# yxtay/transformer-recommenders

Hardware: AMD Instinct MI355X
Metric: user-sequences/sec (train step) MovieLens-1M seq200 d128 @1/2/4/8 GPU (higher is better)
Workload: dtype bf16; 1 GPU; MovieLens-1M-shaped: 3883 items, seq_len=200, d_model=128, 4-layer causal BERT (heads=4, ffn=512), InfoNCELoss over in-batch shared negatives, AdamW; per_gpu_batch=512, global_batch=512, seq_len=200, lengths=dense, loss_heads_evaluated=all 7 + LogitsStatistics (reference training_step), parallelism=dp1, launch=eager launches

## Files before the change

### transformer-recommenders_amd/csrc/common.h

```cpp
#pragma once
#include <hip/hip_runtime.h>
#include <stdint.h>

#include "xfmr_hip.h"

typedef __attribute__((ext_vector_type(8))) __bf16 bf16x8;
typedef __attribute__((ext_vector_type(4))) __bf16 bf16x4;
typedef __attribute__((ext_vector_type(2))) __bf16 bf16x2;
typedef __attribute__((ext_vector_type(16))) float f32x16;

#define XF_WAVE 64

#define XF_LAUNCH_CHECK()                                   \
  do {                                                      \
    if (hipGetLastError() != hipSuccess) return XFMR_EHIP;  \
  } while (0)

static inline bool xf_aligned16(const void* p) { return (reinterpret_cast<uintptr_t>(p) & 15u) == 0; }

__device__ __forceinline__ int xf_lane() { return threadIdx.x & 63; }

__device__ __forceinline__ int xf_acc_row(int r, int lane) { return (r & 3) + 8 * (r >> 2) + 4 * (lane >> 5); }

struct PrecBF16 {
// ... 503 lines not shown
  }
  __device__ static __forceinline__ void tile_xb_tr(f32x16& acc, const __bf16* img, int hsub, int jrow0,
                                                    const f32x16& x) {
    const int l = xf_lane(), g16 = l >> 4, hh = g16 >> 1, li = l & 15, q = li >> 2, p = li & 3;
    const int col = hsub * 32 + 16 * (g16 & 1) + 4 * p;
    const int c = col >> 3, within = col & 7;
#pragma unroll
    for (int s = 0; s < 2; ++s) {
      bf16x8 b;
#pragma unroll
      for (int j = 0; j < 8; ++j) b[j] = (__bf16)x[8 * s + j];
      union { xf_s16x4 v[2]; bf16x8 f; } a;
#pragma unroll
      for (int t = 0; t < 2; ++t) {
        const int row = jrow0 + 16 * s + 8 * t + 4 * hh + q;
        const __bf16* ptr = img + off(row, c) + within;
        a.v[t] = __builtin_amdgcn_ds_read_tr16_b64_v4i16(
            (__attribute__((address_space(3))) xf_s16x4*)(ptr));
      }
      acc = __builtin_amdgcn_mfma_f32_32x32x16_bf16(a.f, b, acc, 0, 0, 0);
    }
  }
  __device__ static __forceinline__ bf16x8 frag_tr(const __bf16* img, int col0, int k0) {
    const int l = xf_lane(), g16 = l >> 4, li = l & 15, q = li >> 2, p = li & 3;
    const int col = col0 + 16 * (g16 & 1) + 4 * p;
    const int c = col >> 3, within = col & 7;
    union { xf_s16x4 v[2]; bf16x8 f; } a;
#pragma unroll
    for (int t = 0; t < 2; ++t) {
      const int row = k0 + 8 * (g16 >> 1) + 4 * t + q;
      a.v[t] = __builtin_amdgcn_ds_read_tr16_b64_v4i16(
          (__attribute__((address_space(3))) xf_s16x4*)(img + off(row, c) + within));
    }
    return a.f;
  }
  __device__ static __forceinline__ int gather_row(int row0) { return row0 + xf_lane() / CPR; }
  __device__ static __forceinline__ int gather_src_chunk(int row) { return (xf_lane() % CPR) ^ swz(row); }
  static constexpr int kRowsPerInstr = 64 / CPR;
};

__device__ __forceinline__ void xf_glds16(const void* gsrc, void* lds_base) {
  __builtin_amdgcn_global_load_lds((const __attribute__((address_space(1))) void*)gsrc,
                                   (__attribute__((address_space(3))) void*)lds_base, 16, 0, 0);
}
__device__ __forceinline__ void xf_glds16_raw_so(const void* sbase, uint32_t voff, void* lds_base) {
  const unsigned dst = (unsigned)(uintptr_t)(__attribute__((address_space(3))) void*)lds_base;
  unsigned keep;
// ... 18 lines not shown
```

### transformer-recommenders_amd/csrc/encoder.hip

```cpp
#include <math.h>
#include <stdlib.h>
#include <new>
#include <string.h>

#include "internal.h"

namespace {

struct LayerParams {
  int64_t wqkv, bqkv, wo, bo, ln1g, ln1b, w1, b1, w2, b2, ln2g, ln2b;
};
struct ParamLayout {
  int64_t pos, type, eg, eb;
  int64_t total;
};

int64_t layer_base(const xfmr_encoder_cfg* c, int i, ParamLayout* pl) {
  const int64_t H = c->hidden, I = c->inter;
  pl->pos = 0;
  pl->type = pl->pos + (int64_t)c->max_pos * H;
  pl->eg = pl->type + 2 * H;
  pl->eb = pl->eg + H;
  const int64_t first = pl->eb + H;
  const int64_t per = 3 * H * H + 3 * H + H * H + H + 2 * H + I * H + I + H * I + H + 2 * H;
// ... 45 lines not shown
size_t up256(size_t x) { return (x + 255) & ~(size_t)255; }

__global__ __launch_bounds__(256) void params_to_bf16_kernel(const float* src, __bf16* dst, int64_t n4) {
  const int64_t i = (int64_t)blockIdx.x * 256 + threadIdx.x;
  if (i < n4) xf_st4<true>(dst, 4 * i, *reinterpret_cast<const float4*>(src + 4 * i));
}

bool mixed_storage(const xfmr_encoder_cfg* c) {
  static const bool force_fp32 = [] {
    const char* e = getenv("XFMR_ACT_FP32");
    return e && *e && *e != '0';
  }();
  return c->precision == XFMR_PREC_BF16 && !force_fp32;
}
int prof(const xfmr_encoder_cfg* c, int kind, int layer, int which, hipStream_t st) {
  if (c->profile_kernel != kind || c->profile_layer != layer || !c->profile_events[which]) return XFMR_OK;
  return hipEventRecord((hipEvent_t)c->profile_events[which], st) == hipSuccess ? XFMR_OK : XFMR_EHIP;
}

struct EncPlan {
  int64_t Tplan, T;
  bool mix, causal;
  bool fuse_ln, fuse_ffn, rederive, fuse_ffn_bwd, dw_buffers_per_layer, dw_side, group_dw, lin_copy;
  int half_layer;
};
constexpr int64_t kDwSideTokens = 40960;
constexpr int64_t kFfnFusedTokens = 16384;
int64_t ln_fused_min_tokens() {
  static const int64_t min_tokens = [] { const char* e = getenv("XFMR_LN_FUSED_MIN_TOKENS"); return e ? (int64_t)atoll(e) : (int64_t)12288; }();
  return min_tokens;
}
EncPlan make_plan(const xfmr_encoder_cfg* c) {
  EncPlan p{};
  const uint32_t f = c->flags;
  p.Tplan = (int64_t)c->batch * c->seq_len;
  p.T = c->seq_offsets ? c->packed_rows : p.Tplan;
  p.mix = mixed_storage(c);
  p.causal = !(f & XFMR_ENC_BIDIRECTIONAL);
  p.fuse_ln = p.mix && c->hidden == 128 && p.Tplan >= ln_fused_min_tokens() && !(f & XFMR_ENC_LN_UNFUSED);
  p.fuse_ffn = p.fuse_ln && p.Tplan >= kFfnFusedTokens && (c->inter % 128) == 0 && c->inter <= 1024 && !(f & XFMR_ENC_FFN_UNFUSED);
  const char* const store_x = getenv("XFMR_LN_STORE_X");
  p.rederive = p.fuse_ln && !(store_x && *store_x && *store_x != '0');
  p.fuse_ffn_bwd = p.fuse_ffn && p.fuse_ln && !(f & XFMR_ENC_FFN_BWD_UNFUSED);
  const bool side_any = (f & XFMR_ENC_DW_SIDE_ANY) != 0;
  p.dw_buffers_per_layer = p.mix && c->layers <= 64 && (side_any || (c->hidden == 128 && p.Tplan >= kDwSideTokens)) &&
                           c->context && !(f & XFMR_ENC_DW_INLINE);
  p.dw_side = p.dw_buffers_per_layer && (side_any || p.T >= kDwSideTokens || !c->seq_offsets);
  p.group_dw = !(f & XFMR_ENC_DW_UNPAIRED) && !p.dw_side && p.mix;
  p.lin_copy = c->hidden_dropout > 0.f || p.mix;
  p.half_layer = ((c->grads_half_event || (f & XFMR_ENC_REDUCE_HALF_EARLY)) && c->layers >= 2) ? c->layers / 2 : -1;
  return p;
}

struct Bump {
  unsigned char* base;
  size_t o;
  void* bytes(size_t n) { void* p = base ? base + o : nullptr; o += up256(n); return p; }
  float* f32(size_t n) { return reinterpret_cast<float*>(bytes(n * sizeof(float))); }
};
struct Workspace {
  Acts a;
  unsigned char* base;
  int layers;
  bool per_layer;
  size_t T, TH, TI, lse, es, xb, slab_w2, slab_w1, slab_wo, slab_wqkv, b1, bqkv, lnrec;
  size_t grads0, grads_stride, red0, red_stride, act0, act_stride;
// ... 221 lines not shown
int xfmr_context_destroy(void* context) {
  if (!context) return XFMR_EINVAL;
  XfContext* c = (XfContext*)context;
  if (c->ev_in) (void)hipEventDestroy(c->ev_in);
  if (c->ev_done) (void)hipEventDestroy(c->ev_done);
  if (c->side) (void)hipStreamDestroy(c->side);
  delete c;
  return XFMR_OK;
}

}

namespace {

struct Residual { const float* x; XfLnResidual re; };

int encoder_forward(const xfmr_encoder_cfg* cfg, const EncPlan& plan, const FwdBufs& a, const float* params,
                    const int64_t* item_idx, const float* table, int64_t n_rows, float* tok, uint8_t* key_mask, hipStream_t st) {
  const int B = cfg->batch, L = cfg->seq_len, H = cfg->hidden, I = cfg->inter, A = cfg->heads;
  const int32_t* const offs = cfg->seq_offsets;
  const int64_t T = plan.T;
  const int prec = cfg->precision;
  const bool mix = plan.mix, keep = a.keep, rederive = plan.rederive && keep;
  const float hdrop = cfg->hidden_dropout, eps = cfg->ln_eps;
  const XfSeed sd(cfg->seed, keep ? cfg->step_device : nullptr);
  ParamLayout pl;
  layer_base(cfg, 0, &pl);
  float* const x0 = rederive ? nullptr : a.x0;
  if (offs) {
    XF_TRY(xf_embed_ln_fwd_packed_ex(item_idx, table, n_rows, params + pl.pos, params + pl.type, params + pl.eg,
                                     params + pl.eb, x0, mix ? a.x0b : nullptr, a.emb_pre, a.emb_mean, a.emb_rstd, key_mask,
                                     T, cfg->row_pos, H, eps, hdrop, sd, SITE_EMB, st));
  } else {
    XF_TRY(xf_embed_ln_fwd_ex(item_idx, table, n_rows, params + pl.pos, params + pl.type, params + pl.eg,
                              params + pl.eb, x0, mix ? a.x0b : nullptr, a.emb_pre, a.emb_mean, a.emb_rstd, key_mask, B,
                              L, H, eps, hdrop, sd, SITE_EMB, st));
  }
  if (cfg->embed_event && hipEventRecord((hipEvent_t)cfg->embed_event, st) != hipSuccess) return XFMR_EHIP;
  Residual x{x0, {a.emb_pre, a.emb_mean, a.emb_rstd, params + pl.eg, params + pl.eb, hdrop, SITE_EMB}};
  const void* xg = mix ? a.x0b : (const void*)a.x0;
  if (mix) {
    const int64_t n4 = pl.total / 4;
    hipLaunchKernelGGL(params_to_bf16_kernel, dim3((unsigned)((n4 + 255) / 256)), dim3(256), 0, st, params,
                       (__bf16*)a.wbf, n4);
    XF_LAUNCH_CHECK();
  }
// ... 15 lines not shown
    float* const sum = keep ? pre : a.ln_tmp;
    XF_TRY(xf_linear_fwd_ex(in, W(w), params + bias, sum, T, H, K, XFMR_EPI_BIAS_DROP_RES, res.x, nullptr, hdrop, sd, site,
                            prec, sA | sB, st));
    return xf_layernorm_fwd_ex(sum, params + gamma, params + beta, y, y16, mean, rstd, T, H, eps, st);
  };
  for (int i = 0; i < cfg->layers; ++i) {
    const LayerActs l = a.layer(i);
    const LayerParams p = layer_params(cfg, i);
    const bool last = i == cfg->layers - 1;
    float* const x1 = rederive ? nullptr : l.x1;
    float* const out = last ? tok : (rederive ? nullptr : l.x2);
    void* const x1b = mix ? l.x1b : nullptr;
    void* const x2b = (mix && !last) ? l.x2b : nullptr;
    XF_TRY(xf_linear_fwd_ex(xg, W(p.wqkv), params + p.bqkv, l.qkv, T, 3 * H, H, XFMR_EPI_BIAS, nullptr, nullptr,
                            0.f, 0, 0, prec, sC | sA | sB, st));
    XF_TRY(prof(cfg, XFMR_PROF_ATTN_FWD, i, 0, st));
    XF_TRY(xf_attn_fwd_ex(l.qkv, key_mask, l.ctx, l.lse, B, L, A, H, cfg->attn_dropout, sd, site_attn(i), prec,
                          mix, plan.causal, st, offs));
    XF_TRY(prof(cfg, XFMR_PROF_ATTN_FWD, i, 1, st));
    XF_TRY(linear_ln(l.ctx, p.wo, p.bo, H, x, site_out(i), p.ln1g, p.ln1b, l.pre1, x1, x1b, l.mean1, l.rstd1));
    XF_TRY(prof(cfg, XFMR_PROF_FFN_FWD, i, 0, st));
    const Residual r1{x1, {l.pre1, l.mean1, l.rstd1, params + p.ln1g, params + p.ln1b, 0.f, 0}};
    if (plan.fuse_ffn) {
      XF_TRY(rederive ? xf_ffn_fwd_fused_re(l.x1b, W(p.w1), params + p.b1, W(p.w2), params + p.b2, l.f1, l.g, l.pre2, T, H,
                                            I, &r1.re, hdrop, sd, site_ffn(i), params + p.ln2g, params + p.ln2b, eps, out,
                                            x2b, l.mean2, l.rstd2, st)
             : !keep  ? xf_ffn_fwd_fused_infer(l.x1b, W(p.w1), params + p.b1, W(p.w2), params + p.b2, T, H, I, r1.x,
                                               params + p.ln2g, params + p.ln2b, eps, out, x2b, st)
                      : xf_ffn_fwd_fused_ex(l.x1b, W(p.w1), params + p.b1, W(p.w2), params + p.b2, l.f1, l.g, l.pre2, T, H,
                                            I, r1.x, hdrop, sd, site_ffn(i), params + p.ln2g, params + p.ln2b, eps, out,
                                            x2b, l.mean2, l.rstd2, st));
    } else {
      const void* const x1g = mix ? (const void*)l.x1b : (const void*)l.x1;
      if (keep)
        XF_TRY(xf_linear_fwd_ex(x1g, W(p.w1), params + p.b1, l.g, T, I, H, XFMR_EPI_BIAS_GELU, nullptr, l.f1, 0.f, 0, 0, prec,
                                sC | sA | sB | XF_AUX_GELU_GRAD, st));
      else
        XF_TRY(xf_linear_gelu_fwd_infer(x1g, W(p.w1), params + p.b1, l.g, T, I, H, prec, sC | sA | sB, st));
      XF_TRY(linear_ln(l.g, p.w2, p.b2, I, r1, site_ffn(i), p.ln2g, p.ln2b, l.pre2, out, x2b, l.mean2, l.rstd2));
    }
    XF_TRY(prof(cfg, XFMR_PROF_FFN_FWD, i, 1, st));
    x = Residual{out, {l.pre2, l.mean2, l.rstd2, params + p.ln2g, params + p.ln2b, 0.f, 0}};
    xg = mix ? (const void*)l.x2b : (const void*)out;
  }
  return XFMR_OK;
}

}

extern "C" {

int xfmr_encoder_fwd(const xfmr_encoder_cfg* cfg, const float* params, const int64_t* item_idx,
// ... 95 lines not shown
                                   mix, nullptr, nullptr, nullptr, T, H, off,
                                   xf_make_dropout(cfg->hidden_dropout, sd, site_ffn(i)), r.ln2, st, &blocks));
      ln_segs(r.ln2, blocks, p.ln2g, p.ln2b, p.b2);
    }
    const void* const dlin_ffn = lin_copy ? gb.dLinF : (const void*)a.dA;
    const void* const dlin_out = lin_copy ? gb.dLinO : (const void*)dX;
    int splits[4] = {0, 0, 0, 0};
    const XfDwItem items[4] = {
        {dlin_ffn, l.g, (int32_t)H, (int32_t)I, r.w2, nullptr, &splits[0]},
        {gb.dI, mix ? (const void*)l.x1b : (const void*)l.x1, (int32_t)I, (int32_t)H, r.w1, r.b1, &splits[1]},
        {dlin_out, l.ctx, (int32_t)H, (int32_t)H, r.wo, nullptr, &splits[2]},
        {gb.dQKV, i > 0 ? (mix ? prev.x2b : (const void*)prev.x2) : (mix ? a.x0b : (const void*)a.x0), (int32_t)(3 * H),
         (int32_t)H, r.wqkv, r.bqkv, &splits[3]}};
    const int64_t dw_w[4] = {p.w2, p.w1, p.wo, p.wqkv}, dw_b[4] = {-1, p.b1, -1, p.bqkv};
    auto dw = [&](int k, bool launch) -> int {
      const XfDwItem& it = items[k];
      if (launch) XF_TRY(xf_linear_bwd_dw_deferred(it.dy, it.x, T, it.N, it.K, prec, sAB, it.slabs, it.bias_part, it.splits, dw_stream()));
      seg(it.slabs, grads + dw_w[k], *it.splits, (int64_t)it.N * it.K, (int64_t)it.N * it.K);
      if (it.bias_part) seg(it.bias_part, grads + dw_b[k], *it.splits, it.N, it.N);
      return XFMR_OK;
    };
    if (!plan.group_dw) XF_TRY(dw(0, true));
    XF_TRY(prof(cfg, XFMR_PROF_FFN_BWD, i, 0, st));
    if (plan.fuse_ffn_bwd) {
      XF_TRY(xf_ffn_bwd_dx_fused_ex(dlin_ffn, W(p.w2), l.f1, W(p.w1), gb.dI, T, H, I, a.dA, l.pre1, l.mean1, l.rstd1,
                                    params + p.ln1g, cfg->hidden_dropout, sd, site_out(i), dX, gb.dLinO, r.ln1,
                                    &blocks, st));
    } else {
      XF_TRY(xf_linear_bwd_dx_ex(dlin_ffn, W(p.w2), gb.dI, T, H, I, nullptr, l.f1, prec,
                                 sA | sC | sP | sB | (plan.fuse_ffn ? 0 : XF_AUX_GELU_GRAD), st));
    }
    if (!plan.group_dw) XF_TRY(dw(1, true));
    if (plan.fuse_ffn_bwd) {
    } else if (fuse_lnb) {
      XF_TRY(xf_linear_bwd_dx_lnbwd_ex(gb.dI, W(p.w1), T, I, H, a.dA, l.pre1, l.mean1, l.rstd1, params + p.ln1g,
                                       cfg->hidden_dropout, sd, site_out(i), dX, gb.dLinO, r.ln1, &blocks, prec,
                                       sA | sB, st));
    } else {
      XF_TRY(xf_linear_bwd_dx_ex(gb.dI, W(p.w1), a.dA, T, I, H, a.dA, nullptr, prec, sA | sB, st));
      XF_TRY(xf_layernorm_bwd_impl(a.dA, l.pre1, l.mean1, l.rstd1, params + p.ln1g, dX, lin_copy ? gb.dLinO : nullptr,
                                   mix, nullptr, nullptr, nullptr, T, H, off,
                                   xf_make_dropout(cfg->hidden_dropout, sd, site_out(i)), r.ln1, st, &blocks));
    }
    XF_TRY(prof(cfg, XFMR_PROF_FFN_BWD, i, 1, st));
    ln_segs(r.ln1, blocks, p.ln1g, p.ln1b, p.bo);
    if (!plan.group_dw) XF_TRY(dw(2, true));
    XF_TRY(xf_linear_bwd_dx_ex(dlin_out, W(p.wo), a.dCtx, T, H, H, nullptr, nullptr, prec, sA | sC | sB, st));
// ... 38 lines not shown
    XF_TRY(xf_layernorm_bwd_impl(dX, a.emb_pre, a.emb_mean, a.emb_rstd, params + pl.eg, a.dA, nullptr, false, nullptr,
                                 nullptr, nullptr, T, H, xf_make_dropout(cfg->hidden_dropout, sd, SITE_EMB), off,
                                 a.emb_ln, st, &blocks));
    ln_segs(a.emb_ln, blocks, pl.eg, pl.eb, -1);
  }
  if (offs) XF_TRY(xf_embed_param_grads_packed(a.dA, grads + pl.pos, grads + pl.type, offs, B, L, H, cfg->max_pos, st));
  else XF_TRY(xfmr_embed_param_grads(a.dA, grads + pl.pos, grads + pl.type, B, L, H, cfg->max_pos, stream));
  return XFMR_OK;
  }();
  if (side_used) {
    if (hipEventRecord(ev_done, side) != hipSuccess || hipStreamWaitEvent(st, ev_done, 0) != hipSuccess) side_rc = XFMR_EHIP;
  }
  if (chain_rc != XFMR_OK) return chain_rc;
  if (side_rc != XFMR_OK) return side_rc;
  XF_TRY(prof(cfg, XFMR_PROF_REDUCE, cfg->profile_layer, 0, st));
  XF_TRY(xf_multi_rowsum(segs, nseg, st));
  XF_TRY(prof(cfg, XFMR_PROF_REDUCE, cfg->profile_layer, 1, st));
  if (cfg->grads_half_event && plan.half_layer < 0 &&
      hipEventRecord((hipEvent_t)cfg->grads_half_event, st) != hipSuccess)
    return XFMR_EHIP;
  return XFMR_OK;
}

int xf_encoder_plan(const xfmr_encoder_cfg* cfg, int32_t out[16]) {
  XF_TRY(check_cfg(cfg));
  if (!out) return XFMR_EINVAL;
  const EncPlan p = make_plan(cfg);
  const int32_t v[16] = {(int32_t)p.Tplan, (int32_t)p.T, p.mix, p.causal, p.fuse_ln, p.fuse_ffn, p.rederive,
                         p.fuse_ffn_bwd, p.dw_buffers_per_layer, p.dw_side, p.group_dw, p.lin_copy, p.half_layer};
  memcpy(out, v, sizeof(v));
  return XFMR_OK;
}

int64_t xfmr_param_half_offset(const xfmr_encoder_cfg* cfg) {
  if (!cfg || cfg->layers <= 0) return XFMR_EINVAL;
  if (cfg->layers < 2) return 0;
  return layer_params(cfg, cfg->layers / 2).wqkv;
}

}
```

### transformer-recommenders_amd/csrc/gemm.hip

```cpp
#include <stdio.h>
#include <stdlib.h>
#include <string.h>

#include <algorithm>
#include <type_traits>

#include "internal.h"

#define XF_PIN_SCALAR(x) asm volatile("" : "+v"(x))
#ifndef XF_LN_DIAG
#define XF_LN_DIAG 0
#endif
#ifndef XF_GEMM_PF
#define XF_GEMM_PF 1
#endif
#ifndef XF_DW_PF
#define XF_DW_PF 1
#endif
#ifdef XF_FFN_STAMP
#define XF_STAMP(i) do { if (stamp_on) st_buf[(i)] = __builtin_readcyclecounter(); } while (0)
#else
#define XF_STAMP(i) do {} while (0)
#endif
#ifndef XF_FFN_ASM_BARRIER
// ... 1157 lines not shown
      XF_LOOP_BARRIER();
      xf_static_for<2>([&](auto ic) {
        constexpr int i = decltype(ic)::value;
        const int p = tid + i * 256, row = p >> 3, ch = p & 7;
        const bf16x8 d8 = di_piece(sF, i);
        if (m0 + row < M) *reinterpret_cast<bf16x8*>(f.DI + (m0 + row) * I + c * CH + ch * 8) = d8;
        *reinterpret_cast<bf16x8*>(sG + row * LDC + ch * 8) = d8;
      });
      commit_w1();
      XF_LOOP_BARRIER();
      if (c + 1 < nchunk) { load_w1(c + 1); load_u(c + 1); }
#pragma unroll
      for (int ks = 0; ks < CH / 16; ++ks) {
        const bf16x8 fa = FN::get(sG, LDC, wr * 32, ks * 16);
#pragma unroll
        for (int j = 0; j < 2; ++j) accx[j] = xf_mma(fa, FT::get(sW, LD2, wc * 64 + j * 32, ks * 16), accx[j]);
      }
    }
    __syncthreads();
    epi_dx_lnbwd_64x128(accx, reinterpret_cast<unsigned char*>(sW), f.e, m0, tix.m, wid, lane);
  }
}

template <class T>
__global__ __launch_bounds__(256) void rowsum_kernel(float* dst, const T* src, int64_t rows, int64_t cols,
                                                     int64_t rows_per) {
  __shared__ float red[4][64];
  const int c = threadIdx.x & 63, rg = threadIdx.x >> 6;
  const int64_t col = (int64_t)blockIdx.x * 64 + c;
  const int64_t r0 = (int64_t)blockIdx.y * rows_per;
  const int64_t r1 = (r0 + rows_per < rows) ? r0 + rows_per : rows;
  float s0 = 0.f, s1 = 0.f, s2 = 0.f, s3 = 0.f;
  if (col < cols) {
    int64_t r = r0 + rg;
    for (; r + 12 < r1; r += 16) {
      s0 += (float)src[r * cols + col];
      s1 += (float)src[(r + 4) * cols + col];
      s2 += (float)src[(r + 8) * cols + col];
      s3 += (float)src[(r + 12) * cols + col];
    }
    for (; r < r1; r += 4) s0 += (float)src[r * cols + col];
  }
  red[rg][c] = (s0 + s1) + (s2 + s3);
  __syncthreads();
  if (rg == 0 && col < cols) dst[(int64_t)blockIdx.y * cols + col] = (red[0][c] + red[1][c]) + (red[2][c] + red[3][c]);
}
// ... 394 lines not shown
  const GemmPlan p = gemm_plan(GemmKey{kGemmFfnBwd, M, H, I, XFMR_PREC_BF16, 0, 1, xf_num_cus()}, gemm_switches());
  if (const int rc = plan_rc(p, xf_aligned16(dy16) && xf_aligned16(w2_16) && xf_aligned16(u16) && xf_aligned16(w1_16) &&
                                    xf_aligned16(di16) && xf_aligned16(dx) && xf_aligned16(ln_x) && xf_aligned16(residual_grad) &&
                                    xf_aligned16(d_lin16) && xf_aligned16(ln_gamma)))
    return rc;
  FfnBwdArgs f{};
  f.DY = (const __bf16*)dy16; f.W2 = (const __bf16*)w2_16; f.U = (const __bf16*)u16; f.W1 = (const __bf16*)w1_16;
  f.DI = (__bf16*)di16; f.I = I;
  GemmArgs& g = f.e;
  g.C = dx; g.ldc = H; g.M = M; g.N = H; g.K = I; g.R = residual_grad;
  g.drop = xf_make_dropout(dropout_p, seed, site);
  g.drop2 = xf_make_dropout(0.f, 0, 0);
  g.ln_gamma = ln_gamma; g.lnb_x = ln_x; g.lnb_mean = ln_mean; g.lnb_rstd = ln_rstd; g.D16 = d_lin16;
  g.lnb_partials = partials;
  set_tiles(g, p);
  *blocks_out = p.records;
  const dim3 grid((unsigned)p.grid), block((unsigned)p.block);
  if (p.ffn_ring) hipLaunchKernelGGL(ffn_bwd_dx_fused_kernel<true>, grid, block, 0, st, f);
  else hipLaunchKernelGGL(ffn_bwd_dx_fused_kernel<false>, grid, block, 0, st, f);
  XF_LAUNCH_CHECK();
  return XFMR_OK;
}

int xf_linear_bwd_dx_ex(const void* dy, const float* w, void* dx, int64_t M, int32_t N, int32_t K,
                        const float* residual_grad, const void* gelu_pre, int32_t precision, uint32_t s16,
                        hipStream_t st) {
  if (!dy || !w || !dx) return XFMR_EINVAL;
  const GemmKey k{gelu_pre ? kGemmDxGelu : kGemmDx, M, N, K, precision, s16, 1, 0};
  const GemmPlan p = gemm_plan(k, gemm_switches_once());
  if (const int rc = plan_rc(p, xf_aligned16(dy) && xf_aligned16(w) && xf_aligned16(dx))) return rc;
  GemmArgs g{};
  g.A = dy; g.B = w; g.C = dx; g.lda = N; g.ldb = K; g.ldc = K; g.M = M; g.N = K; g.K = N; g.k_chunk = 0;
  g.bias = nullptr; g.R = residual_grad; g.P = gelu_pre; g.C2 = nullptr;
  g.aux_grad = (s16 & XF_AUX_GELU_GRAD) != 0;
  g.drop = xf_make_dropout(0.f, 0, 0);
  return launch_tile(p, g, st);
}

int xf_linear_bwd_dx_lnbwd_ex(const void* dy, const float* w, int64_t M, int32_t N, int32_t K,
                              const float* residual_grad, const float* ln_x, const float* ln_mean, const float* ln_rstd,
                              const float* ln_gamma, float dropout_p, XfSeed seed, uint32_t site, float* dx,
                              void* d_lin16, float* partials, int* blocks_out, int32_t precision, uint32_t s16,
                              hipStream_t st, float out_dropout_p, uint32_t out_site) {
  if (!dy || !w || !dx || !ln_x || !ln_mean || !ln_rstd || !ln_gamma || !partials || !blocks_out) return XFMR_EINVAL;
  const GemmKey k{kGemmDxLnBwd, M, N, K, precision, s16, 1, xf_num_cus()};
  const GemmPlan p = gemm_plan(k, gemm_switches_once());
// ... 132 lines not shown
```

### transformer-recommenders_amd/csrc/gemm_plan.inc

```
namespace {

constexpr int kDwMaxSplitCap = 256;

int env_int(const char* name, int dflt) { const char* e = getenv(name); return e ? atoi(e) : dflt; }
char env_first(const char* name) { const char* e = getenv(name); return e ? *e : '\0'; }
bool env_on(const char* name) { const char c = env_first(name); return c && c != '0'; }

int64_t dw_slabs_wanted(int N, int K, int max_split) {
  const int64_t tiles = ((N + 63) / 64) * ((K + 63) / 64);
  int64_t want = (1024 + tiles - 1) / tiles;
  if (want > max_split) want = max_split;
  return want < 1 ? 1 : want;
}
constexpr int kDwSlice = 128;
int dw_split_plan(int64_t M, int N, int K, int max_split, int* k_chunk) {
  const int64_t want = dw_slabs_wanted(N, K, max_split);
  int64_t chunk = (M + want - 1) / want;
  chunk = ((chunk + kDwSlice - 1) / kDwSlice) * kDwSlice;
  if (M >= 4096 && chunk < 256) chunk = 256;
  if (chunk < 64) chunk = 64;
  *k_chunk = (int)chunk;
  return (int)((M + chunk - 1) / chunk);
}
int dw_split_bound(int64_t M, int N, int K) {
// ... 55 lines not shown
    s.dw_ring = env_first("XFMR_DW_RING") != '0';
    s.dwr_tokens = std::max(env_int("XFMR_DWR_TOKENS", 3072), 128);
    s.dwr_minwg = std::max(env_int("XFMR_DWR_MINWG", 64), 1);
    s.ffn_chunk = 64;
    return s;
  }();
  return once;
}
GemmSwitches gemm_switches() {
  GemmSwitches s = gemm_switches_once();
  s.ffn_chunk = env_int("XFMR_FFN_CHUNK", 64) == 64 ? 64 : 128;
  s.ffn_reg_stage = env_on("XFMR_FFN_REG_STAGE");
  return s;
}

GemmPlan gemm_plan(const GemmKey& k, const GemmSwitches& sw) {
  const int64_t M = k.M;
  const int N = k.N, K = k.K;
  const bool bf16 = k.precision == XFMR_PREC_BF16;
  GemmPlan p{};
  p.precision = k.precision;

  if (k.op == kGemmFfnFwd || k.op == kGemmFfnFwdRe || k.op == kGemmFfnBwd) {
    const bool fwd = k.op != kGemmFfnBwd;
    if (M <= 0) return gemm_refuse(XFMR_EINVAL, true);
    if (N != 128 || K <= 0 || (K % (fwd ? 128 : 64)) || (fwd && K > 1024)) return gemm_refuse(XFMR_EUNSUPPORTED, true);
    p.family = fwd ? kGemmFfnFwdKernel : kGemmFfnBwdKernel;
    p.epi = !fwd ? EPI_DX_LNBWD : k.op == kGemmFfnFwdRe ? EPI_DROP_RES_LN_RE : EPI_DROP_RES_LN;
    p.precision = XFMR_PREC_BF16; p.bm = 64; p.bn = 128;
    if (fwd) p.ffn_chunk = sw.ffn_chunk == 64 ? 64 : 128;
    else p.ffn_ring = !sw.ffn_reg_stage;
    if (!whole_row_grid(p, k, sw)) return gemm_refuse(XFMR_EUNSUPPORTED, false);
    if (!fwd) p.records = p.nt_m;
    return p;
  }

  struct OpForm { int epi; uint32_t keep; bool dx; };
  static constexpr OpForm kForms[kGemmFfnFwd] = {
      {EPI_STORE, SABC, false}, {EPI_GELU, SABC, false}, {EPI_DROP_RES, SABC, false},
      {EPI_DROP_RES_LN, SAB, false}, {EPI_DROP_RES_LN_RE, SAB, false}, {EPI_DROP_RES_LN_RED, SAB, false},
      {EPI_STORE, SABCP, true}, {EPI_GELU_GRAD, SABCP, true}, {EPI_DX_LNBWD, SAB, true},
      {EPI_SPLITK, SAB, false}, {EPI_SPLITK, SAB, false}, {EPI_SPLITK, SAB, false}};
  if (k.op < 0 || k.op >= kGemmFfnFwd) return gemm_refuse(XFMR_EINVAL, true);
  const OpForm f = kForms[k.op];
  p.epi = f.epi; p.s16 = k.s16 & f.keep;
  const bool dw = f.epi == EPI_SPLITK, whole_row = epi_res_ln(f.epi) || f.epi == EPI_DX_LNBWD;
  const int64_t gm = dw ? N : M;
  const int gn = (dw || f.dx) ? K : N;
  int kspan = f.dx ? N : K;
  if (whole_row) {
    if (M <= 0 || kspan <= 0) return gemm_refuse(XFMR_EINVAL, true);
    if (gn != 128 || (kspan & 7) || !bf16) return gemm_refuse(XFMR_EUNSUPPORTED, true);
    if (epi_res_mode(f.epi) != 0 && p.s16 != SAB) return gemm_refuse(XFMR_EUNSUPPORTED, false);
  } else {
// ... 55 lines not shown
```

### transformer-recommenders_amd/csrc/internal.h

```cpp
#pragma once
#include "common.h"

enum : uint32_t {
  XF_S16_A = 1u,
  XF_S16_B = 2u,
  XF_S16_C = 4u,
  XF_S16_P = 8u,
  XF_AUX_GELU_GRAD = 0x100u,
};

enum GemmOp : int32_t {
  kGemmFwdBias = 0, kGemmFwdGelu, kGemmFwdDropRes,
  kGemmLnFwd, kGemmLnFwdRe, kGemmLnFwdReDrop,
  kGemmDx, kGemmDxGelu, kGemmDxLnBwd,
  kGemmDw, kGemmDwDeferred, kGemmDwGroup,
  kGemmFfnFwd, kGemmFfnFwdRe, kGemmFfnBwd,
  kGemmOps
};
enum GemmFamily : int32_t {
  kGemmNone = 0,
  kGemmTile,
  kGemmGroup,
  kGemmRing,
  kGemmFfnFwdKernel, kGemmFfnBwdKernel,
};
struct GemmKey {
  GemmOp op;
  int64_t M; int32_t N, K;
  int32_t precision; uint32_t s16;
  int32_t items;
  int32_t cus;
};
struct GemmSwitches {
  int32_t tile_bm, tile_bn, tile_bk, tile_set;
  int32_t dw_bm, dw_bn, dw_tile_set;
  int32_t pad_lds;
  int32_t dw_maxsplit;
  int32_t row_tiles_short;
  int32_t skip_dw;
  int32_t dw_ring;
  int32_t dwr_tokens, dwr_minwg;
  int32_t ffn_chunk;
  int32_t ffn_reg_stage;
};
struct GemmPlan {
  int32_t rc_shape;
  int32_t rc;
// ... 34 lines not shown
  const float* pre; const float* mean; const float* rstd; const float* gamma; const float* beta;
  float dropout_p; uint32_t site;
};
int xf_ffn_fwd_fused_re(const void* x16, const void* w1_16, const float* b1, const void* w2_16, const float* b2,
                        void* u16, void* g16, float* pre, int64_t M, int32_t H, int32_t I, const XfLnResidual* res,
                        float dropout_p, XfSeed seed, uint32_t site, const float* gamma, const float* beta, float eps,
                        float* y, void* y16, float* mean, float* rstd, hipStream_t st);
int xf_linear_ln_fwd_re(const void* x, const float* w, const float* bias, float* pre, int64_t M, int32_t N, int32_t K,
                        const XfLnResidual* res, float dropout_p, XfSeed seed, uint32_t site, const float* gamma,
                        const float* beta, float eps, float* y, void* y16, float* mean, float* rstd, int32_t precision,
                        uint32_t s16, hipStream_t st);
int xf_linear_gelu_fwd_infer(const void* x, const float* w, const float* bias, void* y, int64_t M, int32_t N, int32_t K,
                             int32_t precision, uint32_t s16, hipStream_t st);
int xf_linear_ln_fwd_infer(const void* x, const float* w, const float* bias, int64_t M, int32_t N, int32_t K,
                           const float* residual, const float* gamma, const float* beta, float eps, float* y, void* y16,
                           int32_t precision, uint32_t s16, hipStream_t st);
int xf_ffn_fwd_fused_infer(const void* x16, const void* w1_16, const float* b1, const void* w2_16, const float* b2, int64_t M,
                           int32_t H, int32_t I, const float* residual, const float* gamma, const float* beta, float eps,
                           float* y, void* y16, hipStream_t st);
int xf_ffn_bwd_dx_fused_ex(const void* dy16, const void* w2_16, const void* u16, const void* w1_16, void* di16, int64_t M,
                           int32_t H, int32_t I, const float* residual_grad, const float* ln_x, const float* ln_mean,
                           const float* ln_rstd, const float* ln_gamma, float dropout_p, XfSeed seed, uint32_t site,
                           float* dx, void* d_lin16, float* partials, int* blocks_out, hipStream_t st);
int xf_linear_bwd_dx_ex(const void* dy, const float* w, void* dx, int64_t M, int32_t N, int32_t K,
                        const float* residual_grad, const void* gelu_pre, int32_t precision, uint32_t s16,
                        hipStream_t st);
int xf_linear_bwd_dw_ex(const void* dy, const void* x, float* dw, int64_t M, int32_t N, int32_t K, int32_t precision,
                        void* workspace, size_t workspace_bytes, uint32_t s16, hipStream_t st);
int xf_colsum_ex(const void* a, bool a16, float* out, int64_t M, int32_t N, void* workspace, hipStream_t st);
size_t xf_linear_bwd_dw_slab_bytes(int64_t M, int32_t N, int32_t K);
int xf_linear_bwd_dw_deferred(const void* dy, const void* x, int64_t M, int32_t N, int32_t K, int32_t precision,
                              uint32_t s16, float* slabs, float* bias_part, int* splits, hipStream_t st);
struct XfDwItem { const void* dy; const void* x; int32_t N, K; float* slabs; float* bias_part; int* splits; };
int xf_linear_bwd_dw_group(const XfDwItem* items, int n, int64_t M, int32_t precision, uint32_t s16, hipStream_t st);
int xf_dw_split_plan(int64_t M, int32_t N, int32_t K, int* k_chunk);
bool xf_dw_ring_takes(const XfDwItem* items, int n, int64_t M, int32_t precision, uint32_t s16);
int xf_dw_ring_launch(const XfDwItem* items, int n, int64_t M, hipStream_t st);
int xf_dw_ring_launch_plans(const XfDwItem* items, const GemmPlan* plans, int n, int64_t M, hipStream_t st);
struct XfReduceSeg { const float* src; float* dst; int rows; int cols; int ld; int pad; };
int xf_multi_rowsum(const XfReduceSeg* segs, int nseg, hipStream_t st);
int xf_rowsum(float* dst, const float* src, int64_t rows, int64_t cols, hipStream_t st);
int xf_attn_fwd_ex(const void* qkv, const uint8_t* key_mask, void* ctx, float* lse, int32_t B, int32_t L, int32_t A,
                   int32_t H, float dropout_p, XfSeed seed, uint32_t site, int32_t precision, bool s16,
                   bool causal, hipStream_t st, const int32_t* seq_offsets = nullptr,
                   bool stream_keys = false);
int xf_attn_bwd_ex(const void* qkv, const uint8_t* key_mask, const void* ctx, const float* lse, const void* d_ctx,
// ... 5 lines not shown
int xf_linear_ln_fwd_ex(const void* x, const float* w, const float* bias, float* pre, int64_t M, int32_t N, int32_t K,
                        const float* residual, float dropout_p, XfSeed seed, uint32_t site, const float* gamma,
                        const float* beta, float eps, float* y, void* y16, float* mean, float* rstd, int32_t precision,
                        uint32_t s16, hipStream_t st);
int xf_linear_bwd_dx_lnbwd_ex(const void* dy, const float* w, int64_t M, int32_t N, int32_t K,
                              const float* residual_grad, const float* ln_x, const float* ln_mean, const float* ln_rstd,
                              const float* ln_gamma, float dropout_p, XfSeed seed, uint32_t site, float* dx,
                              void* d_lin16, float* partials, int* blocks_out, int32_t precision, uint32_t s16,
                              hipStream_t st, float out_dropout_p = 0.f, uint32_t out_site = 0);
int xf_ln_row_tiles(int64_t M);
int xf_layernorm_fwd_ex(const float* x, const float* gamma, const float* beta, float* y, void* y16, float* mean,
                        float* rstd, int64_t rows, int32_t H, float eps, hipStream_t stream);
int xf_embed_ln_fwd_ex(const int64_t* item_idx, const float* table, int64_t n_rows, const float* pos_emb,
                       const float* type_emb, const float* gamma, const float* beta, float* out, void* out16,
                       float* pre, float* mean, float* rstd, uint8_t* key_mask, int32_t B, int32_t L, int32_t H,
                       float eps, float dropout_p, XfSeed seed, uint32_t site, hipStream_t stream);
int xf_embed_ln_fwd_packed_ex(const int64_t* item_idx, const float* table, int64_t n_rows, const float* pos_emb,
                              const float* type_emb, const float* gamma, const float* beta, float* out, void* out16,
                              float* pre, float* mean, float* rstd, uint8_t* key_mask, int64_t rows, const int32_t* row_pos,
                              int32_t H, float eps, float dropout_p, XfSeed seed, uint32_t site, hipStream_t stream);
int xf_embed_param_grads_packed(const float* d_pre, float* d_pos, float* d_type, const int32_t* offs, int32_t B, int32_t L,
                                int32_t H, int32_t max_pos, hipStream_t st);
int xf_encoder_plan(const xfmr_encoder_cfg* cfg, int32_t out[16]);
int xf_attn_plan(int32_t bwd, int32_t precision, int32_t s16, int32_t B, int32_t L, int32_t A, int32_t H, int32_t causal,
                 int32_t packed, int32_t stream_keys, int32_t switches, int32_t out[8]);
int xf_attn_switches();
int xf_loss_plan(int64_t T, int32_t H, int64_t n_rows, int32_t train_head, int32_t all_heads, int32_t mask_false_negatives,
                 int32_t mode, int32_t precision, int32_t num_hard_negatives, uint32_t flags, int32_t has_d_tok,
                 int32_t has_table_bf16, int32_t cus, uint64_t switches, int32_t out[40]);
uint64_t xf_loss_switches();
int xf_layernorm_bwd_impl(const float* dy, const float* x, const float* mean, const float* rstd, const float* gamma,
                          float* dx, void* d_lin, bool lin16, float* d_gamma, float* d_beta, float* d_bias,
                          int64_t rows, int32_t H, XfDropout drop_out, XfDropout drop_lin, void* partials,
                          hipStream_t st, int* blocks_out = nullptr);
}
```

Measured before the change: 173,000 sequences/s.

## Recompute FFN pre-activation in fused backward instead of storing it

The fused FFN forward no longer writes the intermediate pre-activation tensor (u = x·W1+b1) when recompute is enabled, which is the default. A new fused backward kernel recomputes u chunk by chunk from the stored LN1 output and W1 inside the dX kernel, then applies the GELU gradient and continues with the dX GEMM. This removes a T×I bf16 write in forward and the matching read in backward, at the cost of an extra GEMM of the same size in backward plus extra W1 staging in shared memory.

```diff
diff --git a/transformer-recommenders_amd/csrc/common.h b/transformer-recommenders_amd/csrc/common.h
--- a/transformer-recommenders_amd/csrc/common.h
+++ b/transformer-recommenders_amd/csrc/common.h
@@ -549,7 +549,10 @@
     }
   }
   __device__ static __forceinline__ bf16x8 frag_tr(const __bf16* img, int col0, int k0) {
-    const int l = xf_lane(), g16 = l >> 4, li = l & 15, q = li >> 2, p = li & 3;
+    return frag_tr(img, col0, k0, xf_lane());
+  }
+  __device__ static __forceinline__ bf16x8 frag_tr(const __bf16* img, int col0, int k0, int l) {
+    const int g16 = l >> 4, li = l & 15, q = li >> 2, p = li & 3;
     const int col = col0 + 16 * (g16 & 1) + 4 * p;
     const int c = col >> 3, within = col & 7;
     union { xf_s16x4 v[2]; bf16x8 f; } a;
diff --git a/transformer-recommenders_amd/csrc/encoder.hip b/transformer-recommenders_amd/csrc/encoder.hip
--- a/transformer-recommenders_amd/csrc/encoder.hip
+++ b/transformer-recommenders_amd/csrc/encoder.hip
@@ -91,6 +91,7 @@
   int64_t Tplan, T;
   bool mix, causal;
   bool fuse_ln, fuse_ffn, rederive, fuse_ffn_bwd, dw_buffers_per_layer, dw_side, group_dw, lin_copy;
+  bool recompute_u;
   int half_layer;
 };
 constexpr int64_t kDwSideTokens = 40960;
@@ -111,6 +112,8 @@
   const char* const store_x = getenv("XFMR_LN_STORE_X");
   p.rederive = p.fuse_ln && !(store_x && *store_x && *store_x != '0');
   p.fuse_ffn_bwd = p.fuse_ffn && p.fuse_ln && !(f & XFMR_ENC_FFN_BWD_UNFUSED);
+  const char* const store_u = getenv("XFMR_FFN_STORE_U");
+  p.recompute_u = p.fuse_ffn_bwd && !(store_u && *store_u && *store_u != '0');
   const bool side_any = (f & XFMR_ENC_DW_SIDE_ANY) != 0;
   p.dw_buffers_per_layer = p.mix && c->layers <= 64 && (side_any || (c->hidden == 128 && p.Tplan >= kDwSideTokens)) &&
                            c->context && !(f & XFMR_ENC_DW_INLINE);
@@ -378,6 +381,7 @@
   const int64_t T = plan.T;
   const int prec = cfg->precision;
   const bool mix = plan.mix, keep = a.keep, rederive = plan.rederive && keep;
+  const bool store_u = !plan.recompute_u;
   const float hdrop = cfg->hidden_dropout, eps = cfg->ln_eps;
   const XfSeed sd(cfg->seed, keep ? cfg->step_device : nullptr);
   ParamLayout pl;
@@ -439,12 +443,13 @@
     XF_TRY(prof(cfg, XFMR_PROF_FFN_FWD, i, 0, st));
     const Residual r1{x1, {l.pre1, l.mean1, l.rstd1, params + p.ln1g, params + p.ln1b, 0.f, 0}};
     if (plan.fuse_ffn) {
-      XF_TRY(rederive ? xf_ffn_fwd_fused_re(l.x1b, W(p.w1), params + p.b1, W(p.w2), params + p.b2, l.f1, l.g, l.pre2, T, H,
+      void* const u = store_u ? l.f1 : nullptr;
+      XF_TRY(rederive ? xf_ffn_fwd_fused_re(l.x1b, W(p.w1), params + p.b1, W(p.w2), params + p.b2, u, l.g, l.pre2, T, H,
                                             I, &r1.re, hdrop, sd, site_ffn(i), params + p.ln2g, params + p.ln2b, eps, out,
                                             x2b, l.mean2, l.rstd2, st)
              : !keep  ? xf_ffn_fwd_fused_infer(l.x1b, W(p.w1), params + p.b1, W(p.w2), params + p.b2, T, H, I, r1.x,
                                                params + p.ln2g, params + p.ln2b, eps, out, x2b, st)
-                      : xf_ffn_fwd_fused_ex(l.x1b, W(p.w1), params + p.b1, W(p.w2), params + p.b2, l.f1, l.g, l.pre2, T, H,
+                      : xf_ffn_fwd_fused_ex(l.x1b, W(p.w1), params + p.b1, W(p.w2), params + p.b2, u, l.g, l.pre2, T, H,
                                             I, r1.x, hdrop, sd, site_ffn(i), params + p.ln2g, params + p.ln2b, eps, out,
                                             x2b, l.mean2, l.rstd2, st));
     } else {
@@ -586,7 +591,11 @@
     };
     if (!plan.group_dw) XF_TRY(dw(0, true));
     XF_TRY(prof(cfg, XFMR_PROF_FFN_BWD, i, 0, st));
-    if (plan.fuse_ffn_bwd) {
+    if (plan.recompute_u) {
+      XF_TRY(xf_ffn_bwd_dx_fused_rc(dlin_ffn, W(p.w2), l.x1b, params + p.b1, W(p.w1), gb.dI, T, H, I, a.dA, l.pre1, l.mean1,
+                                    l.rstd1, params + p.ln1g, cfg->hidden_dropout, sd, site_out(i), dX, gb.dLinO, r.ln1,
+                                    &blocks, st));
+    } else if (plan.fuse_ffn_bwd) {
       XF_TRY(xf_ffn_bwd_dx_fused_ex(dlin_ffn, W(p.w2), l.f1, W(p.w1), gb.dI, T, H, I, a.dA, l.pre1, l.mean1, l.rstd1,
                                     params + p.ln1g, cfg->hidden_dropout, sd, site_out(i), dX, gb.dLinO, r.ln1,
                                     &blocks, st));
@@ -671,13 +680,20 @@
   return XFMR_OK;
 }
 
-int xf_encoder_plan(const xfmr_encoder_cfg* cfg, int32_t out[16]) {
+int xf_encoder_plan_ex(const xfmr_encoder_cfg* cfg, int32_t out[32]) {
   XF_TRY(check_cfg(cfg));
   if (!out) return XFMR_EINVAL;
   const EncPlan p = make_plan(cfg);
-  const int32_t v[16] = {(int32_t)p.Tplan, (int32_t)p.T, p.mix, p.causal, p.fuse_ln, p.fuse_ffn, p.rederive,
-                         p.fuse_ffn_bwd, p.dw_buffers_per_layer, p.dw_side, p.group_dw, p.lin_copy, p.half_layer};
+  const int32_t v[32] = {(int32_t)p.Tplan, (int32_t)p.T, p.mix, p.causal, p.fuse_ln, p.fuse_ffn, p.rederive,
+                         p.fuse_ffn_bwd, p.dw_buffers_per_layer, p.dw_side, p.group_dw, p.lin_copy, p.half_layer,
+                         p.recompute_u};
   memcpy(out, v, sizeof(v));
+  return XFMR_OK;
+}
+int xf_encoder_plan(const xfmr_encoder_cfg* cfg, int32_t out[16]) {
+  int32_t v[32];
+  XF_TRY(xf_encoder_plan_ex(cfg, v));
+  for (int i = 0; i < 16; ++i) out[i] = i < 13 ? v[i] : 0;
   return XFMR_OK;
 }
 
diff --git a/transformer-recommenders_amd/csrc/gemm.hip b/transformer-recommenders_amd/csrc/gemm.hip
--- a/transformer-recommenders_amd/csrc/gemm.hip
+++ b/transformer-recommenders_amd/csrc/gemm.hip
@@ -1203,6 +1203,162 @@
   }
 }
 
+struct FfnBwdRcArgs {
+  const __bf16* DY;
+  const __bf16* W2;
+  const __bf16* X;
+  const float* b1;
+  const __bf16* W1;
+  __bf16* DI;
+  int I;
+  GemmArgs e;
+};
+
+__global__ __launch_bounds__(256, 3) void ffn_bwd_dx_fused_rc_kernel(const FfnBwdRcArgs f_in) {
+  FfnBwdRcArgs f = f_in;
+  XF_CHAIN_PRIO();
+  f.e.drop = xf_drop_resolve(f.e.drop); f.e.drop2 = xf_drop_resolve(f.e.drop2);
+  constexpr int H = 128, BM = 64, CH = 64, LDH = H + 8, LDC = CH + 8;
+  constexpr int EPI_BYTES = (4 * 16 * 68 + 2 * 2 * 2 * 16 * 2 + 2 * 3 * 128) * 4;
+  constexpr int MAX_I = 1024;
+  using FN = Frag<PrecBF16, false>;
+  const int lane = threadIdx.x & 63, wid = threadIdx.x >> 6, tid = threadIdx.x;
+  const int wr = wid >> 1, wc = wid & 1;
+  const TileIdx tix = tile_of(1, f.e.nt_m, 1);
+  if (!tix.valid) return;
+  const int64_t m0 = xf_tile_rows(f.e, tix.m, BM);
+  const int64_t M = f.e.M;
+  const int I = f.I, nchunk = I / CH;
+
+  constexpr int G_BYTES = BM * LDC * 2, W2_BYTES = H * CH * 2, W1_BYTES = CH * H * 2, B1_BYTES = MAX_I * 4;
+  __shared__ __attribute__((aligned(16))) unsigned char smem[W2_BYTES + G_BYTES + W1_BYTES + B1_BYTES];
+  static_assert(BM * LDH * 2 <= G_BYTES + W1_BYTES, "the dy and x tiles are staged over sG and the W1 image");
+  static_assert(EPI_BYTES <= W2_BYTES + G_BYTES, "the epilogue's scratch aliases the W2 image and sG");
+  static_assert(W2_BYTES % 1024 == 0 && G_BYTES % 1024 == 0, "DMA targets on 1-KiB instruction boundaries");
+  __bf16* const sW2 = reinterpret_cast<__bf16*>(smem);
+  __bf16* const sG = reinterpret_cast<__bf16*>(smem + W2_BYTES);
+  __bf16* const sW1 = reinterpret_cast<__bf16*>(smem + W2_BYTES + G_BYTES);
+  float* const sB1 = reinterpret_cast<float*>(smem + W2_BYTES + G_BYTES + W1_BYTES);
+  __bf16* const sY = sG;
+  using I2 = SwzImg<CH>;
+  using I1 = SwzImg<H>;
+  const int w = __builtin_amdgcn_readfirstlane(wid), wrs = w >> 1, wcs = w & 1;
+  auto fresh = [](int v) { asm volatile("" : "+v"(v)); return v; };
+  uint32_t vo2[4], vo1[4];
+  xf_static_for<4>([&](auto jc) {
+    constexpr int j = decltype(jc)::value;
+    const int k2 = I2::gather_row(32 * w + I2::kRowsPerInstr * j), k1 = I1::gather_row(16 * w + I1::kRowsPerInstr * j);
+    vo2[j] = (uint32_t)(k2 * I + 8 * I2::gather_src_chunk(k2)) * 2u;
+    vo1[j] = (uint32_t)(k1 * H + 8 * I1::gather_src_chunk(k1)) * 2u;
+  });
+  auto issue_w2 = [&](int c) {
+    xf_static_for<4>([&](auto jc) {
+      constexpr int j = decltype(jc)::value;
+      xf_glds16_raw_so(f.W2 + c * CH, vo2[j], sW2 + (32 * w + I2::kRowsPerInstr * j) * CH);
+    });
+  };
+  auto issue_w1 = [&](int c) {
+    xf_static_for<4>([&](auto jc) {
+      constexpr int j = decltype(jc)::value;
+      xf_glds16_raw_so(f.W1 + c * (CH * H), vo1[j], sW1 + (16 * w + I1::kRowsPerInstr * j) * H);
+    });
+  };
+  const int prow = tid >> 3, pch = tid & 7;
+  const bool ok0 = m0 + prow < M, ok1 = m0 + prow + 32 < M;
+  __bf16* const di0 = f.DI + (m0 + prow) * I + pch * 8;
+
+  issue_w2(0);
+  bf16x8 ya[H / 16], xa[H / 16];
+  {
+    uint4 yr[4], xr[4];
+#pragma unroll
+    for (int i = 0; i < 4; ++i) {
+      const int p = tid + i * 256, row = p >> 4, ch = p & 15;
+      yr[i] = make_uint4(0u, 0u, 0u, 0u);
+      xr[i] = make_uint4(0u, 0u, 0u, 0u);
+      if (m0 + row < M) {
+        yr[i] = *reinterpret_cast<const uint4*>(f.DY + (m0 + row) * H + ch * 8);
+        xr[i] = *reinterpret_cast<const uint4*>(f.X + (m0 + row) * H + ch * 8);
+      }
+    }
+    for (int i = tid; i < I; i += 256) sB1[i] = f.b1[i];
+#pragma unroll
+    for (int i = 0; i < 4; ++i) {
+      const int p = tid + i * 256, row = p >> 4, ch = p & 15;
+      *reinterpret_cast<uint4*>(sY + row * LDH + ch * 8) = yr[i];
+    }
+    XF_LOOP_BARRIER();
+#pragma unroll
+    for (int ks = 0; ks < H / 16; ++ks) ya[ks] = FN::get(sY, LDH, wr * 32, ks * 16);
+    XF_LOOP_BARRIER();
+#pragma unroll
+    for (int i = 0; i < 4; ++i) {
+      const int p = tid + i * 256, row = p >> 4, ch = p & 15;
+      *reinterpret_cast<uint4*>(sY + row * LDH + ch * 8) = xr[i];
+    }
+    XF_LOOP_BARRIER();
+#pragma unroll
+    for (int ks = 0; ks < H / 16; ++ks) xa[ks] = FN::get(sY, LDH, wr * 32, ks * 16);
+  }
+
+  f32x16 accx[2];
+#pragma unroll
+  for (int j = 0; j < 2; ++j)
+#pragma unroll
+    for (int r = 0; r < 16; ++r) accx[j][r] = 0.f;
+
+  for (int c = 0; c < nchunk; ++c) {
+    xf_wait_vm<0>();
+    XF_LOOP_BARRIER();
+    f32x16 accg, accu;
+#pragma unroll
+    for (int r = 0; r < 16; ++r) { accg[r] = 0.f; accu[r] = 0.f; }
+    {
+      const int l = fresh(lane);
+      issue_w1(c);
+#pragma unroll
+      for (int ks = 0; ks < H / 16; ++ks) accg = xf_mma(ya[ks], I2::frag_tr(sW2, wcs * 32, ks * 16, l), accg);
+    }
+    xf_wait_vm<0>();
+    XF_LOOP_BARRIER();
+    {
+      const int l = fresh(lane);
+      if (c + 1 < nchunk) issue_w2(c + 1);
+      const int rb = wcs * 32 + (l & 31);
+      const int a0 = rb * H + 8 * ((l >> 5) ^ I1::swz(rb));
+#pragma unroll
+      for (int ks = 0; ks < H / 16; ++ks)
+        accu = xf_mma(xa[ks], *reinterpret_cast<const bf16x8*>(sW1 + (a0 ^ (16 * ks))), accu);
+      const int col = wcs * 32 + (l & 31);
+      const float b = sB1[c * CH + col];
+      __bf16* const g = sG + (wrs * 32 + 4 * (l >> 5)) * LDC + col;
+#pragma unroll
+      for (int r = 0; r < 16; ++r) {
+        const __bf16 u = (__bf16)(accu[r] + b);
+        g[((r & 3) + 8 * (r >> 2)) * LDC] = (__bf16)(accg[r] * xf_gelu_grad((float)u));
+      }
+    }
+    XF_LOOP_BARRIER();
+    {
+      const int l = fresh(lane);
+      const int p0 = w * 64 + l;
+      const bf16x8* const src = reinterpret_cast<const bf16x8*>(sG + (p0 >> 3) * LDC + (p0 & 7) * 8);
+      __bf16* const dst = di0 + c * CH;
+      const bf16x8 d0 = src[0], d1 = src[32 * LDC / 8];
+      if (ok0) *reinterpret_cast<bf16x8*>(dst) = d0;
+      if (ok1) *reinterpret_cast<bf16x8*>(dst + (int64_t)32 * I) = d1;
+#pragma unroll
+      for (int ks = 0; ks < CH / 16; ++ks) {
+        const bf16x8 fa = *reinterpret_cast<const bf16x8*>(sG + (wrs * 32 + (l & 31)) * LDC + ks * 16 + 8 * (l >> 5));
+#pragma unroll
+        for (int j = 0; j < 2; ++j) accx[j] = xf_mma(fa, I1::frag_tr(sW1, wcs * 64 + j * 32, ks * 16, l), accx[j]);
+      }
+    }
+  }
+  __syncthreads();
+  epi_dx_lnbwd_64x128(accx, smem, f.e, m0, tix.m, wid, lane);
+}
+
 template <class T>
 __global__ __launch_bounds__(256) void rowsum_kernel(float* dst, const T* src, int64_t rows, int64_t cols,
                                                      int64_t rows_per) {
@@ -1643,6 +1799,34 @@
   return XFMR_OK;
 }
 
+int xf_ffn_bwd_dx_fused_rc(const void* dy16, const void* w2_16, const void* x16, const float* b1, const void* w1_16,
+                           void* di16, int64_t M, int32_t H, int32_t I, const float* residual_grad, const float* ln_x,
+                           const float* ln_mean, const float* ln_rstd, const float* ln_gamma, float dropout_p, XfSeed seed,
+                           uint32_t site, float* dx, void* d_lin16, float* partials, int* blocks_out, hipStream_t st) {
+  if (!dy16 || !w2_16 || !x16 || !b1 || !w1_16 || !di16 || !ln_x || !ln_mean || !ln_rstd || !ln_gamma || !dx || !partials ||
+      !blocks_out)
+    return XFMR_EINVAL;
+  const GemmPlan p = gemm_plan(GemmKey{kGemmFfnBwd, M, H, I, XFMR_PREC_BF16, XF_FFN_RECOMPUTE_U, 1, xf_num_cus()}, gemm_switches());
+  if (const int rc = plan_rc(p, xf_aligned16(dy16) && xf_aligned16(w2_16) && xf_aligned16(x16) && xf_aligned16(w1_16) &&
+                                    xf_aligned16(di16) && xf_aligned16(dx) && xf_aligned16(ln_x) && xf_aligned16(residual_grad) &&
+                                    xf_aligned16(d_lin16) && xf_aligned16(ln_gamma)))
+    return rc;
+  FfnBwdRcArgs f{};
+  f.DY = (const __bf16*)dy16; f.W2 = (const __bf16*)w2_16; f.X = (const __bf16*)x16; f.b1 = b1; f.W1 = (const __bf16*)w1_16;
+  f.DI = (__bf16*)di16; f.I = I;
+  GemmArgs& g = f.e;
+  g.C = dx; g.ldc = H; g.M = M; g.N = H; g.K = I; g.R = residual_grad;
+  g.drop = xf_make_dropout(dropout_p, seed, site);
+  g.drop2 = xf_make_dropout(0.f, 0, 0);
+  g.ln_gamma = ln_gamma; g.lnb_x = ln_x; g.lnb_mean = ln_mean; g.lnb_rstd = ln_rstd; g.D16 = d_lin16;
+  g.lnb_partials = partials;
+  set_tiles(g, p);
+  *blocks_out = p.records;
+  hipLaunchKernelGGL(ffn_bwd_dx_fused_rc_kernel, dim3((unsigned)p.grid), dim3((unsigned)p.block), 0, st, f);
+  XF_LAUNCH_CHECK();
+  return XFMR_OK;
+}
+
 int xf_linear_bwd_dx_ex(const void* dy, const float* w, void* dx, int64_t M, int32_t N, int32_t K,
                         const float* residual_grad, const void* gelu_pre, int32_t precision, uint32_t s16,
                         hipStream_t st) {
diff --git a/transformer-recommenders_amd/csrc/gemm_plan.inc b/transformer-recommenders_amd/csrc/gemm_plan.inc
--- a/transformer-recommenders_amd/csrc/gemm_plan.inc
+++ b/transformer-recommenders_amd/csrc/gemm_plan.inc
@@ -101,14 +101,15 @@
   p.precision = k.precision;
 
   if (k.op == kGemmFfnFwd || k.op == kGemmFfnFwdRe || k.op == kGemmFfnBwd) {
-    const bool fwd = k.op != kGemmFfnBwd;
+    const bool fwd = k.op != kGemmFfnBwd, rc = !fwd && (k.s16 & XF_FFN_RECOMPUTE_U);
     if (M <= 0) return gemm_refuse(XFMR_EINVAL, true);
-    if (N != 128 || K <= 0 || (K % (fwd ? 128 : 64)) || (fwd && K > 1024)) return gemm_refuse(XFMR_EUNSUPPORTED, true);
-    p.family = fwd ? kGemmFfnFwdKernel : kGemmFfnBwdKernel;
+    if (N != 128 || K <= 0 || (K % (fwd ? 128 : 64)) || ((fwd || rc) && K > 1024)) return gemm_refuse(XFMR_EUNSUPPORTED, true);
+    p.family = fwd ? kGemmFfnFwdKernel : rc ? kGemmFfnBwdRcKernel : kGemmFfnBwdKernel;
     p.epi = !fwd ? EPI_DX_LNBWD : k.op == kGemmFfnFwdRe ? EPI_DROP_RES_LN_RE : EPI_DROP_RES_LN;
     p.precision = XFMR_PREC_BF16; p.bm = 64; p.bn = 128;
+    if (rc) p.s16 = XF_FFN_RECOMPUTE_U;
     if (fwd) p.ffn_chunk = sw.ffn_chunk == 64 ? 64 : 128;
-    else p.ffn_ring = !sw.ffn_reg_stage;
+    else p.ffn_ring = rc || !sw.ffn_reg_stage;
     if (!whole_row_grid(p, k, sw)) return gemm_refuse(XFMR_EUNSUPPORTED, false);
     if (!fwd) p.records = p.nt_m;
     return p;
diff --git a/transformer-recommenders_amd/csrc/internal.h b/transformer-recommenders_amd/csrc/internal.h
--- a/transformer-recommenders_amd/csrc/internal.h
+++ b/transformer-recommenders_amd/csrc/internal.h
@@ -7,6 +7,7 @@
   XF_S16_C = 4u,
   XF_S16_P = 8u,
   XF_AUX_GELU_GRAD = 0x100u,
+  XF_FFN_RECOMPUTE_U = 0x200u,
 };
 
 enum GemmOp : int32_t {
@@ -23,6 +24,7 @@
   kGemmGroup,
   kGemmRing,
   kGemmFfnFwdKernel, kGemmFfnBwdKernel,
+  kGemmFfnBwdRcKernel,
 };
 struct GemmKey {
   GemmOp op;
@@ -103,6 +105,10 @@
                            int32_t H, int32_t I, const float* residual_grad, const float* ln_x, const float* ln_mean,
                            const float* ln_rstd, const float* ln_gamma, float dropout_p, XfSeed seed, uint32_t site,
                            float* dx, void* d_lin16, float* partials, int* blocks_out, hipStream_t st);
+int xf_ffn_bwd_dx_fused_rc(const void* dy16, const void* w2_16, const void* x16, const float* b1, const void* w1_16,
+                           void* di16, int64_t M, int32_t H, int32_t I, const float* residual_grad, const float* ln_x,
+                           const float* ln_mean, const float* ln_rstd, const float* ln_gamma, float dropout_p, XfSeed seed,
+                           uint32_t site, float* dx, void* d_lin16, float* partials, int* blocks_out, hipStream_t st);
 int xf_linear_bwd_dx_ex(const void* dy, const float* w, void* dx, int64_t M, int32_t N, int32_t K,
                         const float* residual_grad, const void* gelu_pre, int32_t precision, uint32_t s16,
                         hipStream_t st);
@@ -154,6 +160,7 @@
 int xf_embed_param_grads_packed(const float* d_pre, float* d_pos, float* d_type, const int32_t* offs, int32_t B, int32_t L,
                                 int32_t H, int32_t max_pos, hipStream_t st);
 int xf_encoder_plan(const xfmr_encoder_cfg* cfg, int32_t out[16]);
+int xf_encoder_plan_ex(const xfmr_encoder_cfg* cfg, int32_t out[32]);
 int xf_attn_plan(int32_t bwd, int32_t precision, int32_t s16, int32_t B, int32_t L, int32_t A, int32_t H, int32_t causal,
                  int32_t packed, int32_t stream_keys, int32_t switches, int32_t out[8]);
 int xf_attn_switches();
```

Result: no change. 174,300 sequences/s (median of 6 runs) (+0.8%).
